# preethamam/AutomaticPanoramicImageStitching-AutoPanoStitch-MATLAB

Measured on AMD Instinct MI355X. Metric: MPix/s end-to-end stitch (SIFT->blend), 64x4K images, higher is better.
Workload: dtype f32; 1 GPU

## Files before the change

### automaticpanoramicimagestitching-autopanostitch-matlab_amd/csrc/sift.hip

```cpp
#include <algorithm>
#include <cmath>
#include <cstring>
#include <vector>

#include "aps_internal.h"
#include "select_dev.h"

namespace aps {

constexpr int kBorder = 5;
constexpr int kMaxInterp = 5;
constexpr int kOriBins = 36;
constexpr float kFix = 1048576.0f;

__device__ __forceinline__ long long to_fix(float v) { return (long long)(int)rintf(v * kFix); }
constexpr float kFltEps = 1.1920928955078125e-07f;

constexpr int kMaxViews = APS_SIFT_MAX_VIEWS;
constexpr int kViewShift = 44;
static_assert(kMaxViews <= 16, "the view takes 4 bits of the key");
struct ViewImgs {
    const uint8_t* p[kMaxViews];
};

// ... 195 lines not shown
        const int uc = live ? u : 0;
        const int seg = uc / (IH / 2), p = uc - seg * (IH / 2), xb = seg * 8;
        const f32x2* src = reinterpret_cast<const f32x2*>(&s_in[p * IP2 + 2 * (OFF + xb)]);
        f32x2 v[8 + 2 * R], acc[8];
#pragma unroll
        for (int j = 0; j < 8 + 2 * R; ++j) v[j] = src[j];
#pragma unroll
        for (int j = 0; j < 8; ++j) acc[j] = f32x2{0.f, 0.f};
        static_for<0, 2 * R + 1>([&](auto T) {
            constexpr int t = decltype(T)::value;
#pragma unroll
            for (int j = 0; j < 8; ++j) pk_tap<t>(acc[j], gk, v[j + t]);
        });
        if (one_buf) __syncthreads();
        float* d0 = &s_row[(2 * p) * RPITCH + xb];
        if (live) {
#pragma unroll
            for (int j = 0; j < 8; ++j) {
                d0[j] = acc[j].x;
                d0[RPITCH + j] = acc[j].y;
            }
        }
    }
    __syncthreads();
    for (int u = tid; u < (TW / 2) * (kTH / 4); u += NT) {
        const int lx = 2 * (u & (TW / 2 - 1)), yb = (u / (TW / 2)) * 4;
        f32x2 v[4 + 2 * R], acc[4];
#pragma unroll
        for (int j = 0; j < 4 + 2 * R; ++j) v[j] = *reinterpret_cast<const f32x2*>(&s_row[(yb + j) * RPITCH + lx]);
#pragma unroll
        for (int j = 0; j < 4; ++j) acc[j] = f32x2{0.f, 0.f};
        static_for<0, 2 * R + 1>([&](auto T) {
            constexpr int t = decltype(T)::value;
#pragma unroll
            for (int j = 0; j < 4; ++j) pk_tap<t>(acc[j], gk, v[j + t]);
        });
        const int gx = x0 + lx;
        if (gx + 1 < w && (w & 1) == 0) {
#pragma unroll
            for (int j = 0; j < 4; ++j) {
                const int gy = y0 + yb + j;
                if (gy < h) *reinterpret_cast<f32x2*>(&out[(size_t)gy * w + gx]) = acc[j];
            }
        } else if (gx < w) {
#pragma unroll
            for (int j = 0; j < 4; ++j) {
                const int gy = y0 + yb + j;
                if (gy < h) {
                    out[(size_t)gy * w + gx] = acc[j].x;
                    if (gx + 1 < w) out[(size_t)gy * w + gx + 1] = acc[j].y;
                }
            }
        }
        if (dec && (gx >> 1) < dw) {
#pragma unroll
            for (int j = 0; j < 4; j += 2) {
                const int dy = (y0 + yb + j) >> 1;
                if (dy < dh) dec[(size_t)dy * dw + (gx >> 1)] = acc[j].x;
            }
        }
    }
}

template <int R, int TW = kTW, int NT = 256>
__global__ __launch_bounds__(NT) void blur_kernel(const float* __restrict__ in_, int h, int w, GaussK gk,
                                                   float* __restrict__ out_, float* __restrict__ dec_, int dh, int dw,
                                                   size_t pitch, size_t dpitch) {
    const float* __restrict__ in = in_ + blockIdx.z * pitch;
    float* __restrict__ out = out_ + blockIdx.z * pitch;
    float* __restrict__ dec = dec_ ? dec_ + blockIdx.z * dpitch : nullptr;
    constexpr int RP = (R + 3) & ~3;
    constexpr int IW = TW + 2 * RP, IH = kTH + 2 * R, NV = IW / 4;
    static_assert(IH % 2 == 0 && kTH % 4 == 0, "row pairs");
    constexpr int IP2 = 2 * IW + 4;
    constexpr int RPITCH = TW + 2;
    static_assert((IP2 / 4) % 2 == 1, "pitch");
    static_assert(IH * RPITCH <= (IH / 2) * IP2, "the row-pass result fits the tile's buffer");
    __shared__ __attribute__((aligned(16))) float s_in[(IH / 2) * IP2];
    __shared__ __attribute__((aligned(16))) float s_row_own[kBlurOneBuffer<R> ? 1 : IH * RPITCH];
    float* const s_row = kBlurOneBuffer<R> ? s_in : s_row_own;
    const int x0 = blockIdx.x * TW, y0 = blockIdx.y * kTH;
    const int tid = threadIdx.x;
    const bool vec_ok = (w & 3) == 0 && (reinterpret_cast<uintptr_t>(in) & 15) == 0;
    constexpr int NPF = (IH * NV + NT - 1) / NT;
    float4 pf[NPF];
    const bool interior = vec_ok && x0 >= RP && x0 + TW + RP <= w && y0 >= R && y0 + kTH + R <= h;
    if (interior) {
        const float* base = in + ((size_t)(y0 - R) * w + (x0 - RP));
#pragma unroll
        for (int q = 0; q < NPF; ++q) {
            const int e = tid + NT * q;
            const int ec = e < IH * NV ? e : IH * NV - 1;
            const int ly = ec / NV, v = ec - ly * NV;
            pf[q] = *reinterpret_cast<const float4*>(base + (unsigned)(ly * w + 4 * v));
        }
    } else {
#pragma unroll
        for (int q = 0; q < NPF; ++q) {
            const int e = tid + NT * q;
            const int ec = e < IH * NV ? e : IH * NV - 1;
            const int ly = ec / NV, v = ec - ly * NV;
            const int gy = reflect101(y0 + ly - R, h), gx = x0 - RP + 4 * v;
            const float* row = in + (size_t)gy * w;
            if (vec_ok && gx >= 0 && gx + 3 < w) {
                pf[q] = *reinterpret_cast<const float4*>(row + gx);
            } else {
                pf[q].x = row[reflect101(gx, w)];
                pf[q].y = row[reflect101(gx + 1, w)];
                pf[q].z = row[reflect101(gx + 2, w)];
                pf[q].w = row[reflect101(gx + 3, w)];
            }
        }
    }
#pragma unroll
    for (int q = 0; q < NPF; ++q) {
        const int e = tid + NT * q;
        if (e < IH * NV) {
            const int ly = e / NV, v = e - ly * NV;
            float* dst = &s_in[(ly >> 1) * IP2 + 8 * v + (ly & 1)];
            dst[0] = pf[q].x;
            dst[2] = pf[q].y;
            dst[4] = pf[q].z;
            dst[6] = pf[q].w;
        }
    }
    blur_tile_passes<R, TW, NT>(s_in, s_row, gk, x0, y0, h, w, out, dec, dh, dw);
}

__global__ __launch_bounds__(256) void gray_u8_kernel(ViewImgs imgs, int h, int w, int c, int layout,
                                                      uint8_t* __restrict__ gray_, size_t gpitch) {
    const uint8_t* __restrict__ img = imgs.p[blockIdx.z];
    uint8_t* __restrict__ gray = gray_ + blockIdx.z * gpitch;
    const int x4 = (blockIdx.x * 256 + threadIdx.x) * 4, y = blockIdx.y;
    if (x4 >= w) return;
    uint8_t g[4];
    const bool fast = c == 3 && layout == APS_IMG_U8_HWC && (w & 3) == 0 && (reinterpret_cast<uintptr_t>(img) & 3) == 0;
    if (fast) {
        const uint32_t* p = reinterpret_cast<const uint32_t*>(img + ((size_t)y * w + x4) * 3);
        const uint32_t a = p[0], b = p[1], d_ = p[2];
        const uint8_t ch[12] = {(uint8_t)a, (uint8_t)(a >> 8), (uint8_t)(a >> 16), (uint8_t)(a >> 24), (uint8_t)b, (uint8_t)(b >> 8),
                                (uint8_t)(b >> 16), (uint8_t)(b >> 24), (uint8_t)d_, (uint8_t)(d_ >> 8), (uint8_t)(d_ >> 16), (uint8_t)(d_ >> 24)};
#pragma unroll
        for (int k = 0; k < 4; ++k) {
            const double d = 0.298936021293775 * ch[3 * k] + 0.587043074451121 * ch[3 * k + 1] + 0.114020904255103 * ch[3 * k + 2];
            g[k] = (uint8_t)(float)floor(d + 0.5);
        }
        *reinterpret_cast<uint32_t*>(gray + (size_t)y * w + x4) = g[0] | ((uint32_t)g[1] << 8) | ((uint32_t)g[2] << 16) | ((uint32_t)g[3] << 24);
        return;
    }
    for (int k = 0; k < 4 && x4 + k < w; ++k) {
        const int x = x4 + k;
        float v;
        if (c == 1) {
            v = (float)(layout == APS_IMG_U8_HWC ? img[(size_t)y * w + x] : img[(size_t)x * h + y]);
        } else {
            uint8_t ch[3];
#pragma unroll
            for (int q = 0; q < 3; ++q)
                ch[q] = layout == APS_IMG_U8_HWC ? img[((size_t)y * w + x) * 3 + q] : img[(size_t)q * h * w + (size_t)x * h + y];
            const double d = 0.298936021293775 * ch[0] + 0.587043074451121 * ch[1] + 0.114020904255103 * ch[2];
            v = (float)floor(d + 0.5);
        }
        gray[(size_t)y * w + x] = (uint8_t)v;
    }
}

template <int R>
__global__ __launch_bounds__(256) void blur_base_kernel(const uint8_t* __restrict__ gray_, size_t gpitch, int sh, int sw,
                                                        GaussK gk, float* __restrict__ out_, size_t pitch) {
    const uint8_t* __restrict__ gray = gray_ + blockIdx.z * gpitch;
    float* __restrict__ out = out_ + blockIdx.z * pitch;
    constexpr int RP = (R + 3) & ~3;
    constexpr int IW = kTW + 2 * RP, IH = kTH + 2 * R, NV = IW / 4;
    constexpr int IP2 = 2 * IW + 4;
    constexpr int RPITCH = kTW + 2;
    constexpr int GW = IW / 2 + 3, GH = IH / 2 + 3;
    __shared__ __attribute__((aligned(16))) float s_in[(IH / 2) * IP2];
    __shared__ __attribute__((aligned(16))) float s_row_own[kBlurOneBuffer<R> ? 1 : IH * RPITCH];
    float* const s_row = kBlurOneBuffer<R> ? s_in : s_row_own;
    __shared__ float s_g[GH][GW + 1];
    static_assert(GH * IW <= IH * RPITCH && IW % 4 == 0, "the horizontally interpolated gray rows fit the row-pass buffer");
    __shared__ __attribute__((aligned(16))) float s_h_own[kBlurOneBuffer<R> ? GH * IW : 4];
    const int h = 2 * sh, w = 2 * sw;
    const int x0 = blockIdx.x * kTW, y0 = blockIdx.y * kTH;
    const int tid = threadIdx.x;
    const int lo_x = max(x0 - RP, 0), lo_y = max(y0 - R, 0);
    const int cx0 = max((lo_x + 1) / 2 - 1, 0), cy0 = max((lo_y + 1) / 2 - 1, 0);
    for (int e = tid; e < GH * GW; e += 256) {
        const int ly = e / GW, lx = e - ly * GW;
        const int y = min(cy0 + ly, sh - 1), x = min(cx0 + lx, sw - 1);
        s_g[ly][lx] = (float)gray[(size_t)y * sw + x];
    }
    __shared__ int s_ci[IW + IH][2];
    __shared__ float s_cf[IW + IH];
    if (tid < IW + IH) {
        const bool col = tid < IW;
        const int n = col ? sw : sh, c0 = col ? cx0 : cy0, lim = col ? GW : GH;
        const int p = col ? reflect101(x0 - RP + tid, w) : reflect101(y0 + (tid - IW) - R, h);
        float f = ((float)p + 0.5f) * 0.5f - 0.5f;
        int s0 = (int)floorf(f);
        f -= (float)s0;
        if (s0 < 0) {
            s0 = 0;
            f = 0;
        }
        if (s0 >= n - 1) {
            s0 = n - 1;
            f = 0;
        }
        const int s1 = s0 + 1 < n ? s0 + 1 : n - 1;
        s_ci[tid][0] = min(max(s0 - c0, 0), lim - 1);
        s_ci[tid][1] = min(max(s1 - c0, 0), lim - 1);
        s_cf[tid] = f;
    }
    __syncthreads();
    float* const s_h = kBlurOneBuffer<R> ? s_h_own : s_row;
    for (int e = tid; e < GH * IW; e += 256) {
        const int gy = e / IW, cx = e - gy * IW;
        const float a1 = s_cf[cx], a0 = 1.0f - a1;
        const float* r = s_g[gy];
        s_h[gy * IW + cx] = r[s_ci[cx][0]] * a0 + r[s_ci[cx][1]] * a1;
    }
    __syncthreads();
    for (int e = tid; e < IH * NV; e += 256) {
        const int ly = e / NV, v = e - ly * NV;
        const float b1 = s_cf[IW + ly], b0 = 1.0f - b1;
        const float4 h0 = *reinterpret_cast<const float4*>(&s_h[s_ci[IW + ly][0] * IW + 4 * v]);
        const float4 h1 = *reinterpret_cast<const float4*>(&s_h[s_ci[IW + ly][1] * IW + 4 * v]);
        float* dst = &s_in[(ly >> 1) * IP2 + 8 * v + (ly & 1)];
        dst[0] = h0.x * b0 + h1.x * b1;
        dst[2] = h0.y * b0 + h1.y * b1;
        dst[4] = h0.z * b0 + h1.z * b1;
        dst[6] = h0.w * b0 + h1.w * b1;
    }
    blur_tile_passes<R>(s_in, s_row, gk, x0, y0, h, w, out, nullptr, 0, 0);
}

__global__ void blur_row_generic(const float* __restrict__ in_, int h, int w, GaussK gk, float* __restrict__ out_, size_t pitch) {
    const float* __restrict__ in = in_ + blockIdx.z * pitch;
    float* __restrict__ out = out_ + blockIdx.z * pitch;
    const int x = blockIdx.x * blockDim.x + threadIdx.x, y = blockIdx.y;
    if (x >= w) return;
    const int r = gk.n / 2;
    float acc = 0.f;
    for (int t = 0; t < gk.n; ++t) acc = fmaf(gk.k[t], in[(size_t)y * w + reflect101(x + t - r, w)], acc);
    out[(size_t)y * w + x] = acc;
}
__global__ void blur_col_generic(const float* __restrict__ tmp_, int h, int w, GaussK gk, float* __restrict__ out_, size_t pitch) {
    const float* __restrict__ tmp = tmp_ + blockIdx.z * pitch;
    float* __restrict__ out = out_ + blockIdx.z * pitch;
    const int x = blockIdx.x * blockDim.x + threadIdx.x, y = blockIdx.y;
    if (x >= w) return;
    const int r = gk.n / 2;
    float acc = 0.f;
    for (int t = 0; t < gk.n; ++t) acc = fmaf(gk.k[t], tmp[(size_t)reflect101(y + t - r, h) * w + x], acc);
    out[(size_t)y * w + x] = acc;
}

struct OctaveDesc {
    const float* G[8];
    int w, h;
};

struct KpRec {
    unsigned long long key;
    float xc, xr, xi, contr;
};

#define AT(L, rr, cc) (od.G[(L) + 1][(size_t)(rr) * w + (cc)] - od.G[(L)][(size_t)(rr) * w + (cc)])

__device__ bool adjust_extremum(const OctaveDesc& od, int nl, int o, int layer, int r, int c, float contr_thr,
                                float edge_thr, KpRec& kp) {
    const int w = od.w, h = od.h;
    const float img_scale = 1.0f / 255.0f, deriv_scale = img_scale * 0.5f, second_scale = img_scale,
                cross_scale = img_scale * 0.25f;
    float xi = 0, xr = 0, xc = 0;
    int i = 0;
    for (; i < kMaxInterp; ++i) {
        const int im = layer, pv = layer - 1, nx = layer + 1;
        const float dD0 = (AT(im, r, c + 1) - AT(im, r, c - 1)) * deriv_scale;
        const float dD1 = (AT(im, r + 1, c) - AT(im, r - 1, c)) * deriv_scale;
        const float dD2 = (AT(nx, r, c) - AT(pv, r, c)) * deriv_scale;
        const float v2 = AT(im, r, c) * 2.0f;
        const float dxx = (AT(im, r, c + 1) + AT(im, r, c - 1) - v2) * second_scale;
        const float dyy = (AT(im, r + 1, c) + AT(im, r - 1, c) - v2) * second_scale;
        const float dss = (AT(nx, r, c) + AT(pv, r, c) - v2) * second_scale;
        const float dxy = (AT(im, r + 1, c + 1) - AT(im, r + 1, c - 1) - AT(im, r - 1, c + 1) + AT(im, r - 1, c - 1)) * cross_scale;
        const float dxs = (AT(nx, r, c + 1) - AT(nx, r, c - 1) - AT(pv, r, c + 1) + AT(pv, r, c - 1)) * cross_scale;
        const float dys = (AT(nx, r + 1, c) - AT(nx, r - 1, c) - AT(pv, r + 1, c) + AT(pv, r - 1, c)) * cross_scale;
        float A[3][4] = {{dxx, dxy, dxs, dD0}, {dxy, dyy, dys, dD1}, {dxs, dys, dss, dD2}};
        bool singular = false;
#pragma unroll
        for (int col = 0; col < 3; ++col) {
            if (singular) break;
            int piv = col;
#pragma unroll
            for (int row = col + 1; row < 3; ++row)
                if (fabsf(A[row][col]) > fabsf(A[piv][col])) piv = row;
            if (fabsf(A[piv][col]) < kFltEps) {
                singular = true;
                break;
            }
            if (piv != col) {
#pragma unroll
                for (int e = 0; e < 4; ++e) {
                    const float t = A[piv][e];
                    A[piv][e] = A[col][e];
                    A[col][e] = t;
                }
            }
            const float d = -1.0f / A[col][col];
#pragma unroll
            for (int row = col + 1; row < 3; ++row) {
                const float alpha = A[row][col] * d;
#pragma unroll
                for (int e = col + 1; e < 4; ++e) A[row][e] = fmaf(alpha, A[col][e], A[row][e]);
            }
// ... 176 lines not shown
        for (int p = 0; p < ND; ++p) {
#pragma unroll
            for (int k = 0; k < 2; ++k) {
                wmax[p % 3][k] = fmaxf(fmaxf(hm[a][p][k], hm[b][p][k]), hm[c][p][k]);
                wmin[p % 3][k] = fminf(fminf(hn[a][p][k], hn[b][p][k]), hn[c][p][k]);
            }
            if (p < 2) continue;
            const int layer = p - 1;
#pragma unroll
            for (int k = 0; k < 2; ++k) {
                const float val = dc[b][layer - 1][k];
                const float mx = fmaxf(fmaxf(wmax[0][k], wmax[1][k]), wmax[2][k]);
                const float mn = fminf(fminf(wmin[0][k], wmin[1][k]), wmin[2][k]);
                const bool pass = (k ? ok1 : ok0) && fabsf(val) > thr && ((val > 0 && val >= mx) || (val < 0 && val <= mn));
                emit(pass, layer, r, c0 + k);
            }
        }
    };
    using I0 = std::integral_constant<int, 0>;
    using I1 = std::integral_constant<int, 1>;
    using I2 = std::integral_constant<int, 2>;
    fetch(I0{}, rc0 - 1);
    fetch(I1{}, rc0);
    fetch(I2{}, rc0 + 1);
    reduce_row(I0{});
    fetch(I0{}, rc0 + 2);
    reduce_row(I1{});
    fetch(I1{}, rc0 + 3);
    for (int r = rc0; r < rc1; r += 3) {
        reduce_row(I2{});
        fetch(I2{}, r + 4);
        test_row(I0{}, I1{}, I2{}, r);
        if (r + 1 >= rc1) break;
        reduce_row(I0{});
        fetch(I0{}, r + 5);
        test_row(I1{}, I2{}, I0{}, r + 1);
        if (r + 2 >= rc1) break;
        reduce_row(I1{});
        fetch(I1{}, r + 6);
        test_row(I2{}, I0{}, I1{}, r + 2);
    }
    if (qn == 0) return;
    const int n_loc = min(qn, kWCells);
    unsigned int base = 0;
    if (lane == 0) base = atomicAdd(count, (unsigned int)n_loc);
    base = __builtin_amdgcn_readfirstlane(base);
    __builtin_amdgcn_wave_barrier();
    for (int e = lane; e < n_loc; e += 64) {
        const unsigned int slot = base + e;
        if (slot < cap) cells[slot] = s_cells[wave][e];
    }
}

__global__ void refine_kernel(const PyrTable* __restrict__ pt, const unsigned long long* __restrict__ cells,
                              const unsigned int* __restrict__ n_cells, unsigned int cells_cap, float contr_thr,
                              float edge_thr, KpRec* __restrict__ recs, unsigned int* __restrict__ count,
                              unsigned int cap) {
    const unsigned int i = blockIdx.x * blockDim.x + threadIdx.x, view = blockIdx.y;
    const unsigned int n = min(n_cells[2 * view], cells_cap);
    if (i >= n) return;
    const unsigned long long key = cells[(size_t)view * cells_cap + i];
    const int o = key_octave(key), layer = (int)((key >> 32) & 0xff), r = (int)((key >> 16) & 0xffff),
              c = (int)(key & 0xffff);
    KpRec kp;
    if (!adjust_extremum(pt[view].oct[o], pt[view].nl, o, layer, r, c, contr_thr, edge_thr, kp)) return;
    kp.key |= (unsigned long long)view << kViewShift;
    const unsigned int slot = atomicAdd(count + 2 * view, 1u);
    if (slot < cap) recs[(size_t)view * cap + slot] = kp;
}

__device__ __forceinline__ float kp_scale(float sigma, int layer, float xi, int nl) {
    return sigma * my_exp2(((float)layer + xi) / (float)nl);
}

__global__ __launch_bounds__(256) void orient_kernel(const PyrTable* __restrict__ pt,
                                                     const KpRec* __restrict__ kps, unsigned int n,
                                                     unsigned int* __restrict__ ori_count,
                                                     float* __restrict__ ori_angle ,
                                                     unsigned char* __restrict__ ori_bin ) {
    __shared__ unsigned long long s_hist[4][kOriBins];
    __shared__ float s_h[4][kOriBins + 4];
    const int wv = threadIdx.x >> 6, lane = threadIdx.x & 63;
    const unsigned int ki = blockIdx.x * 4 + wv;
    const bool active = ki < n;
    if (lane < kOriBins) s_hist[wv][lane] = 0ull;
    __syncthreads();
    int o = 0, layer = 1, r0 = 0, c0 = 0, view = 0;
    float xi = 0;
    if (active) {
        const KpRec kp = kps[ki];
        view = key_view(kp.key);
        o = key_octave(kp.key);
        layer = (int)((kp.key >> 32) & 0xff);
        r0 = (int)((kp.key >> 16) & 0xffff);
        c0 = (int)(kp.key & 0xffff);
        xi = kp.xi;
    }
    pt += view;
    const OctaveDesc& od = pt->oct[o];
    const __attribute__((address_space(1))) float* g = (const __attribute__((address_space(1))) float*)od.G[layer];
    const int w = od.w, h = od.h;
    const float scl = kp_scale(pt->sigma, layer, xi, pt->nl);
    const int radius = (int)rintf(4.5f * scl);
    const float sig = 1.5f * scl;
    const float expf_scale = -1.0f / (2.0f * sig * sig);
    const int side = 2 * radius + 1;
    if (active) {
        for (int s = lane; s < side * side; s += 64) {
            const int i = s / side - radius, j = s % side - radius;
            const int y = r0 + i, x = c0 + j;
            if (y <= 0 || y >= h - 1 || x <= 0 || x >= w - 1) continue;
            const int ctr = y * w + x;
            const float dx = g[ctr + 1] - g[ctr - 1];
            const float dy = g[ctr - w] - g[ctr + w];
            const float wgt = my_exp((float)(i * i + j * j) * expf_scale);
            const float ori = fast_atan2_deg(dy, dx);
            const float mag = sqrtf(dx * dx + dy * dy);
            int bin = (int)rintf(((float)kOriBins / 360.0f) * ori);
            if (bin >= kOriBins) bin -= kOriBins;
            if (bin < 0) bin += kOriBins;
            const long long q = to_fix(wgt * mag);
            atomicAdd(&s_hist[wv][bin], (unsigned long long)q);
        }
    }
    __syncthreads();
    if (lane < kOriBins) s_h[wv][lane + 2] = (float)(long long)s_hist[wv][lane] * (1.0f / kFix);
    __syncthreads();
    if (lane < 2) {
        s_h[wv][lane] = s_h[wv][kOriBins + lane];
        s_h[wv][kOriBins + 2 + lane] = s_h[wv][2 + lane];
    }
    __syncthreads();
    float hv = 0.f;
    if (lane < kOriBins)
        hv = (s_h[wv][lane] + s_h[wv][lane + 4]) * (1.0f / 16.0f) + (s_h[wv][lane + 1] + s_h[wv][lane + 3]) * (4.0f / 16.0f) +
             s_h[wv][lane + 2] * (6.0f / 16.0f);
    __syncthreads();
    if (lane < kOriBins) s_h[wv][lane] = hv;
    __syncthreads();
    if (active) {
        float omax = lane < kOriBins ? s_h[wv][lane] : -INFINITY;
#pragma unroll
        for (int off = 32; off > 0; off >>= 1) omax = fmaxf(omax, __shfl_xor(omax, off));
        const float thr = omax * 0.8f;
        bool peak = false;
        float angle = 0.f;
        if (lane < kOriBins) {
            const int j = lane;
            const int l = j > 0 ? j - 1 : kOriBins - 1, r2 = j < kOriBins - 1 ? j + 1 : 0;
            const float hj = s_h[wv][j], hl = s_h[wv][l], hr = s_h[wv][r2];
            if (hj > hl && hj > hr && hj >= thr) {
                peak = true;
                float bin = (float)j + 0.5f * (hl - hr) / (hl - 2.0f * hj + hr);
                bin = bin < 0 ? (float)kOriBins + bin : (bin >= (float)kOriBins ? bin - (float)kOriBins : bin);
                angle = 360.0f - (360.0f / (float)kOriBins) * bin;
                if (fabsf(angle - 360.0f) < kFltEps) angle = 0.0f;
            }
        }
        const unsigned long long pm = __ballot(peak);
        if (peak) {
            const unsigned int cnt = (unsigned int)__popcll(pm & ((1ull << lane) - 1ull));
            ori_angle[(size_t)ki * kOriBins + cnt] = angle;
            ori_bin[(size_t)ki * kOriBins + cnt] = (unsigned char)lane;
        }
        if (lane == 0) ori_count[ki] = (unsigned int)__popcll(pm);
    }
}

struct OrientedKp {
    unsigned int kp;
    float angle;
};

__global__ void expand_oriented_kernel(const unsigned int* __restrict__ ori_count,
                                       const unsigned int* __restrict__ ori_pos,
                                       const float* __restrict__ ori_angle, unsigned int n,
                                       OrientedKp* __restrict__ out) {
    const unsigned int i = blockIdx.x * blockDim.x + threadIdx.x;
    if (i >= n) return;
    const unsigned int c = ori_count[i], p = ori_pos[i];
    for (unsigned int e = 0; e < c; ++e) {
        out[p + e].kp = i;
        out[p + e].angle = ori_angle[(size_t)i * kOriBins + e];
    }
}

__device__ __forceinline__ float octave_step(int o) { return ldexpf(1.0f, o) * 0.5f; }
__device__ __forceinline__ float sift_pt(int base, float offset) { return (float)base + offset; }
__device__ __forceinline__ double sift_loc(float pt, float step) { return (double)(pt * step) + 1.0; }

__global__ __launch_bounds__(256) void sift_contr_key_kernel(const KpRec* __restrict__ kps, const OrientedKp* __restrict__ oks,
                                                             unsigned int n, unsigned long long* __restrict__ keys,
                                                             unsigned int* __restrict__ vals) {
    const unsigned int i = blockIdx.x * 256 + threadIdx.x;
    if (i >= n) return;
    keys[i] = strength_key_f32(kps[oks[i].kp].contr);
    vals[i] = i;
}

__global__ __launch_bounds__(256) void sift_uniform_key_kernel(const KpRec* __restrict__ kps, const OrientedKp* __restrict__ oks,
                                                               unsigned int n, int H, int W, int rows, int cols,
                                                               unsigned long long* __restrict__ keys, unsigned int* __restrict__ vals) {
    const unsigned int i = blockIdx.x * 256 + threadIdx.x;
    if (i >= n) return;
    const KpRec kp = kps[oks[i].kp];
    const float step = octave_step(key_octave(kp.key));
    const double x = sift_loc(sift_pt((int)(kp.key & 0xffff), kp.xc), step), y = sift_loc(sift_pt((int)((kp.key >> 16) & 0xffff), kp.xr), step);
    const int px = min(max((int)floor(x) - 1, 0), W - 1), py = min(max((int)floor(y) - 1, 0), H - 1);
    keys[i] = (unsigned long long)uniform_cell(py, px, H, W, rows, cols) << kSegmentShift | strength_key_f32(kp.contr);
    vals[i] = i;
}

struct ViewDst {
    float* desc;
    double* loc;
    float* aux;
    unsigned int row0;
};
constexpr int kD = 4, kN = 8, kHistLen = (kD + 2) * (kD + 2) * (kN + 2);
constexpr int kDescQueue = 512;

__global__ __launch_bounds__(256) void descr_kernel(const PyrTable* __restrict__ pt,
                                                    const KpRec* __restrict__ kps,
                                                    const OrientedKp* __restrict__ oks, unsigned int n_out,
                                                    const ViewDst* __restrict__ dst, int desc_layout, int64_t ldd, int64_t ldl) {
    __shared__ unsigned long long s_hist[4][kHistLen];
    __shared__ __attribute__((aligned(16))) float s_raw[4][128];
    __shared__ int s_queue[4][kDescQueue];
    const int wv = threadIdx.x >> 6, lane = threadIdx.x & 63;
    const unsigned int oi = blockIdx.x * 4 + wv;
    const bool active = oi < n_out;
    for (int e = lane; e < kHistLen; e += 64) s_hist[wv][e] = 0ull;
    __syncthreads();
    int o = 0, layer = 1, r0 = 0, c0 = 0, view = 0;
    float xc = 0, xr = 0, xi = 0, contr = 0, kangle = 0;
    if (active) {
        const OrientedKp ok = oks[oi];
        const KpRec kp = kps[ok.kp];
        view = key_view(kp.key);
        o = key_octave(kp.key);
        layer = (int)((kp.key >> 32) & 0xff);
        r0 = (int)((kp.key >> 16) & 0xffff);
        c0 = (int)(kp.key & 0xffff);
        xc = kp.xc;
        xr = kp.xr;
        xi = kp.xi;
        contr = kp.contr;
        kangle = ok.angle;
    }
    pt += view;
    const OctaveDesc& od = pt->oct[o];
    const __attribute__((address_space(1))) float* g = (const __attribute__((address_space(1))) float*)od.G[layer];
    const int w = od.w, h = od.h;
    const float scl = kp_scale(pt->sigma, layer, xi, pt->nl);
    float ori = 360.0f - kangle;
    if (fabsf(ori - 360.0f) < kFltEps) ori = 0.0f;
    const float ptx = sift_pt(c0, xc), pty = sift_pt(r0, xr);
    const int px = (int)rintf(ptx), py = (int)rintf(pty);
    float sin_t, cos_t;
    sincos_deg(ori, sin_t, cos_t);
    const float bins_per_deg = (float)kN / 360.0f;
    const float exp_scale = -1.0f / ((float)(kD * kD) * 0.5f);
    const float hist_width = 3.0f * scl;
    int radius = (int)rintf(hist_width * 1.4142135623730951f * (float)(kD + 1) * 0.5f);
    const int diag = (int)sqrt((double)w * w + (double)h * h);
    if (radius > diag) radius = diag;
    cos_t = cos_t / hist_width;
    sin_t = sin_t / hist_width;
    const int side = 2 * radius + 1;
    (void)side;
    auto accumulate = [&](int i, int j) __attribute__((always_inline)) {
        const float c_rot = (float)j * cos_t - (float)i * sin_t;
        const float r_rot = (float)j * sin_t + (float)i * cos_t;
        float rbin = r_rot + (float)(kD / 2) - 0.5f;
        float cbin = c_rot + (float)(kD / 2) - 0.5f;
        const int r = py + i, c = px + j;
        const int ctr = r * w + c;
        const float dx = g[ctr + 1] - g[ctr - 1];
        const float dy = g[ctr - w] - g[ctr + w];
        const float wgt = my_exp((c_rot * c_rot + r_rot * r_rot) * exp_scale);
        const float o_deg = fast_atan2_deg(dy, dx);
        const float mag = sqrtf(dx * dx + dy * dy) * wgt;
        float obin = (o_deg - ori) * bins_per_deg;
        const int rr0 = (int)floorf(rbin), cc0 = (int)floorf(cbin);
        int o0 = (int)floorf(obin);
        rbin -= (float)rr0;
        cbin -= (float)cc0;
        obin -= (float)o0;
        if (o0 < 0) o0 += kN;
        if (o0 >= kN) o0 -= kN;
        const float v_r1 = mag * rbin, v_r0 = mag - v_r1;
        const float v_rc11 = v_r1 * cbin, v_rc10 = v_r1 - v_rc11;
        const float v_rc01 = v_r0 * cbin, v_rc00 = v_r0 - v_rc01;
        const float v111 = v_rc11 * obin, v110 = v_rc11 - v111;
        const float v101 = v_rc10 * obin, v100 = v_rc10 - v101;
        const float v011 = v_rc01 * obin, v010 = v_rc01 - v011;
        const float v001 = v_rc00 * obin, v000 = v_rc00 - v001;
        const int idx = ((rr0 + 1) * (kD + 2) + cc0 + 1) * (kN + 2) + o0;
        unsigned long long* hb = &s_hist[wv][idx];
#define ADDQ(off, v) atomicAdd(hb + (off), (unsigned long long)to_fix(v))
        ADDQ(0, v000);
        ADDQ(1, v001);
        ADDQ(kN + 2, v010);
        ADDQ(kN + 3, v011);
        ADDQ((kD + 2) * (kN + 2), v100);
        ADDQ((kD + 2) * (kN + 2) + 1, v101);
        ADDQ((kD + 3) * (kN + 2), v110);
        ADDQ((kD + 3) * (kN + 2) + 1, v111);
#undef ADDQ
    };
    if (active) {
        int* q = s_queue[wv];
        int qn = 0;
        auto flush = [&]() __attribute__((always_inline)) {
            const int rounds = (qn + 63) >> 6;
            __builtin_amdgcn_wave_barrier();
            const int e0 = lane * rounds;
            int pk = q[min(e0, kDescQueue - 1)];
            for (int r = 0; r < rounds; ++r) {
                const int e = e0 + r;
                const int pk_next = q[min(e + 1, kDescQueue - 1)];
                if (e < qn) accumulate(pk >> 16, (int)(short)(pk & 0xffff));
                pk = pk_next;
            }
            __builtin_amdgcn_wave_barrier();
            qn = 0;
        };
        auto passes = [&](int i, int j) __attribute__((always_inline)) {
            const float c_rot = (float)j * cos_t - (float)i * sin_t;
            const float r_rot = (float)j * sin_t + (float)i * cos_t;
            const float rbin = r_rot + (float)(kD / 2) - 0.5f;
            const float cbin = c_rot + (float)(kD / 2) - 0.5f;
            const int r = py + i, c = px + j;
            return j >= -radius && j <= radius && rbin > -1 && rbin < kD && cbin > -1 && cbin < kD && r > 0 && r < h - 1 && c > 0 && c < w - 1;
        };
        bool plain = radius > 63 || fabsf(sin_t) < 1e-4f || fabsf(cos_t) < 1e-4f;
        int jl_[2] = {0, 0}, len_[2] = {0, 0};
        if (!plain) {
            bool bad = false;
#pragma unroll
            for (int half = 0; half < 2; ++half) {
                const int i = -radius + lane + 64 * half;
                const bool row_ok = i <= radius && py + i > 0 && py + i < h - 1;
                const float fi = (float)i;
                float lo = fmaxf(-(float)radius, (float)(1 - px)), hi = fminf((float)radius, (float)(w - 2 - px));
                auto clip = [&](float a, float lo_v, float hi_v) __attribute__((always_inline)) {
                    const float p0 = lo_v / a, p1 = hi_v / a;
                    lo = fmaxf(lo, fminf(p0, p1));
                    hi = fminf(hi, fmaxf(p0, p1));
                };
                clip(sin_t, -2.5f - fi * cos_t, 2.5f - fi * cos_t);
                clip(cos_t, -2.5f + fi * sin_t, 2.5f + fi * sin_t);
                const int gl = (int)ceilf(lo), gh = (int)floorf(hi);
                int jl = 0x7fffffff, jh = -0x7fffffff;
#pragma unroll
                for (int dlt = 2; dlt >= -2; --dlt)
                    if (passes(i, gl + dlt)) jl = gl + dlt;
#pragma unroll
                for (int dlt = -2; dlt <= 2; ++dlt)
                    if (passes(i, gh + dlt)) jh = gh + dlt;
                const bool none = jl > jh;
                bool good;
                if (none)
                    good = gl > gh;
                else
                    good = !passes(i, jl - 1) && !passes(i, jh + 1) && passes(i, (jl + jh) / 2) && jl >= gl - 2 && jh <= gh + 2;
                bad = bad || (row_ok && !good);
                jl_[half] = jl;
                len_[half] = (row_ok && !none) ? jh - jl + 1 : 0;
            }
            plain = __any(bad) != 0;
        }
        if (!plain) {
#pragma unroll
            for (int half = 0; half < 2; ++half) {
                unsigned long long rows_m = __ballot(len_[half] > 0);
                while (rows_m) {
                    const int l = __ffsll((long long)rows_m) - 1;
                    rows_m &= rows_m - 1ull;
                    const int rj = __builtin_amdgcn_readlane(jl_[half], l), rn = __builtin_amdgcn_readlane(len_[half], l);
                    const int ri = -radius + l + 64 * half;
                    for (int t0 = 0; t0 < rn; t0 += 64) {
                        const int cnt = min(64, rn - t0);
                        if (lane < cnt) q[qn + lane] = (ri << 16) | ((rj + t0 + lane) & 0xffff);
                        qn += cnt;
                        if (qn > kDescQueue - 64) flush();
                    }
                }
            }
        } else {
            for (int i = -radius; i <= radius; ++i) {
                for (int j0 = -radius; j0 <= radius; j0 += 64) {
                    const int j = j0 + lane;
                    const bool pass = passes(i, j);
                    const unsigned long long m = __ballot(pass);
                    if (m == 0ull) continue;
                    if (pass) q[qn + __popcll(m & ((1ull << lane) - 1ull))] = (i << 16) | (j & 0xffff);
                    qn += __popcll(m);
                    if (qn > kDescQueue - 64) flush();
                }
            }
        }
        if (qn > 0) flush();
    }
    __syncthreads();
#pragma unroll
    for (int half = 0; half < 2; ++half) {
        const int e = lane + 64 * half;
        const int k = e & 7, ij = e >> 3, i = ij >> 2, j = ij & 3;
        const int idx = ((i + 1) * (kD + 2) + (j + 1)) * (kN + 2);
        long long v = (long long)s_hist[wv][idx + k];
        if (k < 2) v += (long long)s_hist[wv][idx + kN + k];
        s_raw[wv][e] = (float)v * (1.0f / kFix);
    }
    __syncthreads();
    if (!active) return;
    auto sumsq = [&]() __attribute__((always_inline)) {
        float a = 0;
#pragma unroll 4
        for (int k4 = 0; k4 < 32; ++k4) {
            const float4 v = *reinterpret_cast<const float4*>(&s_raw[wv][4 * k4]);
            a = fmaf(v.x, v.x, a);
            a = fmaf(v.y, v.y, a);
            a = fmaf(v.z, v.z, a);
            a = fmaf(v.w, v.w, a);
        }
        return a;
    };
    float nrm2 = sumsq();
    const float thr = sqrtf(nrm2) * 0.2f;
    float clip[2];
#pragma unroll
    for (int half = 0; half < 2; ++half) {
        const float v0 = s_raw[wv][lane + 64 * half];
        clip[half] = v0 < thr ? v0 : thr;
    }
    __builtin_amdgcn_wave_barrier();
    s_raw[wv][lane] = clip[0];
    s_raw[wv][lane + 64] = clip[1];
    __builtin_amdgcn_wave_barrier();
    nrm2 = sumsq();
    const float sn = sqrtf(nrm2);
    const float scale = 512.0f / (sn > kFltEps ? sn : kFltEps);
    float qv[2];
#pragma unroll
    for (int half = 0; half < 2; ++half) {
        float v = rintf(clip[half] * scale);
        qv[half] = v < 0 ? 0 : (v > 255 ? 255 : v);
    }
    __builtin_amdgcn_wave_barrier();
    s_raw[wv][lane] = qv[0];
    s_raw[wv][lane + 64] = qv[1];
    __builtin_amdgcn_wave_barrier();
    const float qq = sumsq();
    const float inv = sqrtf(qq);
    const ViewDst vd = dst[view];
    const size_t row = oi - vd.row0;
    __attribute__((address_space(1))) float* desc = (__attribute__((address_space(1))) float*)vd.desc;
#pragma unroll
    for (int half = 0; half < 2; ++half) {
        const int e = lane + 64 * half;
        const float outv = inv > 0 ? qv[half] / inv : 0.0f;
        if (desc_layout == APS_ROWMAJOR)
            desc[row * ldd + e] = outv;
        else
            desc[(size_t)e * ldd + row] = outv;
    }
    if (lane == 0) {
        const float s = octave_step(o);
        vd.loc[row] = sift_loc(ptx, s);
        vd.loc[ldl + row] = sift_loc(pty, s);
        if (vd.aux) {
            vd.aux[row * 4 + 0] = scl * s * 2.0f;
            vd.aux[row * 4 + 1] = kangle;
            vd.aux[row * 4 + 2] = contr;
            vd.aux[row * 4 + 3] = (float)(o + 256 * layer);
        }
    }
}

static GaussK make_gauss(double sigma) {
    GaussK g;
    int n = (int)std::lrint(sigma * 8.0 + 1.0) | 1;
    if (n > 63) n = 63;
    const double s2 = -0.5 / (sigma * sigma);
    double sum = 0;
    for (int i = 0; i < n; ++i) {
        const double x = i - (n - 1) * 0.5;
        g.k[i] = (float)std::exp(s2 * x * x);
        sum += g.k[i];
    }
    sum = 1.0 / sum;
    for (int i = 0; i < n; ++i) g.k[i] = (float)(g.k[i] * sum);
    g.n = n;
    return g;
}

static size_t view_pitch(int w, int h) { return ((size_t)w * h + 3) & ~(size_t)3; }

// ... 453 lines not shown
```

Baseline: 3291 MPix/s.

## Pair-row tile loads, fast interior upsample, wave-local barriers in SIFT kernels

```diff
diff --git a/automaticpanoramicimagestitching-autopanostitch-matlab_amd/csrc/sift.hip b/automaticpanoramicimagestitching-autopanostitch-matlab_amd/csrc/sift.hip
--- a/automaticpanoramicimagestitching-autopanostitch-matlab_amd/csrc/sift.hip
+++ b/automaticpanoramicimagestitching-autopanostitch-matlab_amd/csrc/sift.hip
@@ -301,46 +301,47 @@
     const int x0 = blockIdx.x * TW, y0 = blockIdx.y * kTH;
     const int tid = threadIdx.x;
     const bool vec_ok = (w & 3) == 0 && (reinterpret_cast<uintptr_t>(in) & 15) == 0;
-    constexpr int NPF = (IH * NV + NT - 1) / NT;
-    float4 pf[NPF];
+    constexpr int NIT = (IH / 2) * NV, NPF = (NIT + NT - 1) / NT;
+    float4 pa[NPF], pb[NPF];
     const bool interior = vec_ok && x0 >= RP && x0 + TW + RP <= w && y0 >= R && y0 + kTH + R <= h;
     if (interior) {
         const float* base = in + ((size_t)(y0 - R) * w + (x0 - RP));
 #pragma unroll
         for (int q = 0; q < NPF; ++q) {
             const int e = tid + NT * q;
-            const int ec = e < IH * NV ? e : IH * NV - 1;
-            const int ly = ec / NV, v = ec - ly * NV;
-            pf[q] = *reinterpret_cast<const float4*>(base + (unsigned)(ly * w + 4 * v));
+            const int ec = e < NIT ? e : NIT - 1;
+            const int p = ec / NV, v = ec - p * NV;
+            const unsigned off = (unsigned)(2 * p * w + 4 * v);
+            pa[q] = *reinterpret_cast<const float4*>(base + off);
+            pb[q] = *reinterpret_cast<const float4*>(base + (off + (unsigned)w));
         }
     } else {
 #pragma unroll
         for (int q = 0; q < NPF; ++q) {
             const int e = tid + NT * q;
-            const int ec = e < IH * NV ? e : IH * NV - 1;
-            const int ly = ec / NV, v = ec - ly * NV;
-            const int gy = reflect101(y0 + ly - R, h), gx = x0 - RP + 4 * v;
-            const float* row = in + (size_t)gy * w;
+            const int ec = e < NIT ? e : NIT - 1;
+            const int p = ec / NV, v = ec - p * NV;
+            const int gx = x0 - RP + 4 * v;
+            const float* row_a = in + (size_t)reflect101(y0 + 2 * p - R, h) * w;
+            const float* row_b = in + (size_t)reflect101(y0 + 2 * p + 1 - R, h) * w;
             if (vec_ok && gx >= 0 && gx + 3 < w) {
-                pf[q] = *reinterpret_cast<const float4*>(row + gx);
+                pa[q] = *reinterpret_cast<const float4*>(row_a + gx);
+                pb[q] = *reinterpret_cast<const float4*>(row_b + gx);
             } else {
-                pf[q].x = row[reflect101(gx, w)];
-                pf[q].y = row[reflect101(gx + 1, w)];
-                pf[q].z = row[reflect101(gx + 2, w)];
-                pf[q].w = row[reflect101(gx + 3, w)];
+                const int g0 = reflect101(gx, w), g1 = reflect101(gx + 1, w), g2 = reflect101(gx + 2, w), g3 = reflect101(gx + 3, w);
+                pa[q] = make_float4(row_a[g0], row_a[g1], row_a[g2], row_a[g3]);
+                pb[q] = make_float4(row_b[g0], row_b[g1], row_b[g2], row_b[g3]);
             }
         }
     }
 #pragma unroll
     for (int q = 0; q < NPF; ++q) {
         const int e = tid + NT * q;
-        if (e < IH * NV) {
-            const int ly = e / NV, v = e - ly * NV;
-            float* dst = &s_in[(ly >> 1) * IP2 + 8 * v + (ly & 1)];
-            dst[0] = pf[q].x;
-            dst[2] = pf[q].y;
-            dst[4] = pf[q].z;
-            dst[6] = pf[q].w;
+        if (e < NIT) {
+            const int p = e / NV, v = e - p * NV;
+            float4* dst = reinterpret_cast<float4*>(&s_in[p * IP2 + 8 * v]);
+            dst[0] = make_float4(pa[q].x, pb[q].x, pa[q].y, pb[q].y);
+            dst[1] = make_float4(pa[q].z, pb[q].z, pa[q].w, pb[q].w);
         }
     }
     blur_tile_passes<R, TW, NT>(s_in, s_row, gk, x0, y0, h, w, out, dec, dh, dw);
@@ -412,7 +413,8 @@
     }
     __shared__ int s_ci[IW + IH][2];
     __shared__ float s_cf[IW + IH];
-    if (tid < IW + IH) {
+    const bool interior = x0 >= RP && x0 + kTW + RP < w && y0 >= R && y0 + kTH + R < h;
+    if (!interior && tid < IW + IH) {
         const bool col = tid < IW;
         const int n = col ? sw : sh, c0 = col ? cx0 : cy0, lim = col ? GW : GH;
         const int p = col ? reflect101(x0 - RP + tid, w) : reflect101(y0 + (tid - IW) - R, h);
@@ -434,24 +436,52 @@
     }
     __syncthreads();
     float* const s_h = kBlurOneBuffer<R> ? s_h_own : s_row;
-    for (int e = tid; e < GH * IW; e += 256) {
-        const int gy = e / IW, cx = e - gy * IW;
-        const float a1 = s_cf[cx], a0 = 1.0f - a1;
-        const float* r = s_g[gy];
-        s_h[gy * IW + cx] = r[s_ci[cx][0]] * a0 + r[s_ci[cx][1]] * a1;
-    }
-    __syncthreads();
-    for (int e = tid; e < IH * NV; e += 256) {
-        const int ly = e / NV, v = e - ly * NV;
-        const float b1 = s_cf[IW + ly], b0 = 1.0f - b1;
-        const float4 h0 = *reinterpret_cast<const float4*>(&s_h[s_ci[IW + ly][0] * IW + 4 * v]);
-        const float4 h1 = *reinterpret_cast<const float4*>(&s_h[s_ci[IW + ly][1] * IW + 4 * v]);
-        float* dst = &s_in[(ly >> 1) * IP2 + 8 * v + (ly & 1)];
-        dst[0] = h0.x * b0 + h1.x * b1;
-        dst[2] = h0.y * b0 + h1.y * b1;
-        dst[4] = h0.z * b0 + h1.z * b1;
-        dst[6] = h0.w * b0 + h1.w * b1;
-    }
+    const int ry = y0 - R - 1 - 2 * cy0;
+    auto interpolate = [&](auto INTERIOR) __attribute__((always_inline)) {
+        auto terms = [&](int k, int u, int& i0, int& i1, float& f1) __attribute__((always_inline)) {
+            if constexpr (decltype(INTERIOR)::value) {
+                i0 = u >> 1;
+                i1 = i0 + 1;
+                f1 = (u & 1) ? 0.75f : 0.25f;
+            } else {
+                i0 = s_ci[k][0];
+                i1 = s_ci[k][1];
+                f1 = s_cf[k];
+            }
+        };
+        for (int e = tid; e < GH * IW; e += 256) {
+            const int gy = e / IW, cx = e - gy * IW;
+            int i0, i1;
+            float a1;
+            terms(cx, cx + 1, i0, i1, a1);
+            const float a0 = 1.0f - a1;
+            const float* r = s_g[gy];
+            s_h[gy * IW + cx] = r[i0] * a0 + r[i1] * a1;
+        }
+        __syncthreads();
+        for (int e = tid; e < (IH / 2) * NV; e += 256) {
+            const int p = e / NV, v = e - p * NV;
+            float4 res[2];
+#pragma unroll
+            for (int half = 0; half < 2; ++half) {
+                const int ly = 2 * p + half;
+                int j0, j1;
+                float b1;
+                terms(IW + ly, ly + ry, j0, j1, b1);
+                const float b0 = 1.0f - b1;
+                const float4 h0 = *reinterpret_cast<const float4*>(&s_h[j0 * IW + 4 * v]);
+                const float4 h1 = *reinterpret_cast<const float4*>(&s_h[j1 * IW + 4 * v]);
+                res[half] = make_float4(h0.x * b0 + h1.x * b1, h0.y * b0 + h1.y * b1, h0.z * b0 + h1.z * b1, h0.w * b0 + h1.w * b1);
+            }
+            float4* dst = reinterpret_cast<float4*>(&s_in[p * IP2 + 8 * v]);
+            dst[0] = make_float4(res[0].x, res[1].x, res[0].y, res[1].y);
+            dst[1] = make_float4(res[0].z, res[1].z, res[0].w, res[1].w);
+        }
+    };
+    if (interior)
+        interpolate(std::true_type{});
+    else
+        interpolate(std::false_type{});
     blur_tile_passes<R>(s_in, s_row, gk, x0, y0, h, w, out, nullptr, 0, 0);
 }
 
@@ -794,20 +824,13 @@
     __shared__ float s_h[4][kOriBins + 4];
     const int wv = threadIdx.x >> 6, lane = threadIdx.x & 63;
     const unsigned int ki = blockIdx.x * 4 + wv;
-    const bool active = ki < n;
+    if (ki >= n) return;
     if (lane < kOriBins) s_hist[wv][lane] = 0ull;
-    __syncthreads();
-    int o = 0, layer = 1, r0 = 0, c0 = 0, view = 0;
-    float xi = 0;
-    if (active) {
-        const KpRec kp = kps[ki];
-        view = key_view(kp.key);
-        o = key_octave(kp.key);
-        layer = (int)((kp.key >> 32) & 0xff);
-        r0 = (int)((kp.key >> 16) & 0xffff);
-        c0 = (int)(kp.key & 0xffff);
-        xi = kp.xi;
-    }
+    __builtin_amdgcn_wave_barrier();
+    const KpRec kp = kps[ki];
+    const int view = key_view(kp.key), o = key_octave(kp.key), layer = (int)((kp.key >> 32) & 0xff);
+    const int r0 = (int)((kp.key >> 16) & 0xffff), c0 = (int)(kp.key & 0xffff);
+    const float xi = kp.xi;
     pt += view;
     const OctaveDesc& od = pt->oct[o];
     const __attribute__((address_space(1))) float* g = (const __attribute__((address_space(1))) float*)od.G[layer];
@@ -817,66 +840,62 @@
     const float sig = 1.5f * scl;
     const float expf_scale = -1.0f / (2.0f * sig * sig);
     const int side = 2 * radius + 1;
-    if (active) {
-        for (int s = lane; s < side * side; s += 64) {
-            const int i = s / side - radius, j = s % side - radius;
-            const int y = r0 + i, x = c0 + j;
-            if (y <= 0 || y >= h - 1 || x <= 0 || x >= w - 1) continue;
-            const int ctr = y * w + x;
-            const float dx = g[ctr + 1] - g[ctr - 1];
-            const float dy = g[ctr - w] - g[ctr + w];
-            const float wgt = my_exp((float)(i * i + j * j) * expf_scale);
-            const float ori = fast_atan2_deg(dy, dx);
-            const float mag = sqrtf(dx * dx + dy * dy);
-            int bin = (int)rintf(((float)kOriBins / 360.0f) * ori);
-            if (bin >= kOriBins) bin -= kOriBins;
-            if (bin < 0) bin += kOriBins;
-            const long long q = to_fix(wgt * mag);
-            atomicAdd(&s_hist[wv][bin], (unsigned long long)q);
-        }
-    }
-    __syncthreads();
+    for (int s = lane; s < side * side; s += 64) {
+        const int i = s / side - radius, j = s % side - radius;
+        const int y = r0 + i, x = c0 + j;
+        if (y <= 0 || y >= h - 1 || x <= 0 || x >= w - 1) continue;
+        const int ctr = y * w + x;
+        const float dx = g[ctr + 1] - g[ctr - 1];
+        const float dy = g[ctr - w] - g[ctr + w];
+        const float wgt = my_exp((float)(i * i + j * j) * expf_scale);
+        const float ori = fast_atan2_deg(dy, dx);
+        const float mag = sqrtf(dx * dx + dy * dy);
+        int bin = (int)rintf(((float)kOriBins / 360.0f) * ori);
+        if (bin >= kOriBins) bin -= kOriBins;
+        if (bin < 0) bin += kOriBins;
+        const long long q = to_fix(wgt * mag);
+        atomicAdd(&s_hist[wv][bin], (unsigned long long)q);
+    }
+    __builtin_amdgcn_wave_barrier();
     if (lane < kOriBins) s_h[wv][lane + 2] = (float)(long long)s_hist[wv][lane] * (1.0f / kFix);
-    __syncthreads();
+    __builtin_amdgcn_wave_barrier();
     if (lane < 2) {
         s_h[wv][lane] = s_h[wv][kOriBins + lane];
         s_h[wv][kOriBins + 2 + lane] = s_h[wv][2 + lane];
     }
-    __syncthreads();
+    __builtin_amdgcn_wave_barrier();
     float hv = 0.f;
     if (lane < kOriBins)
         hv = (s_h[wv][lane] + s_h[wv][lane + 4]) * (1.0f / 16.0f) + (s_h[wv][lane + 1] + s_h[wv][lane + 3]) * (4.0f / 16.0f) +
              s_h[wv][lane + 2] * (6.0f / 16.0f);
-    __syncthreads();
+    __builtin_amdgcn_wave_barrier();
     if (lane < kOriBins) s_h[wv][lane] = hv;
-    __syncthreads();
-    if (active) {
-        float omax = lane < kOriBins ? s_h[wv][lane] : -INFINITY;
-#pragma unroll
-        for (int off = 32; off > 0; off >>= 1) omax = fmaxf(omax, __shfl_xor(omax, off));
-        const float thr = omax * 0.8f;
-        bool peak = false;
-        float angle = 0.f;
-        if (lane < kOriBins) {
-            const int j = lane;
-            const int l = j > 0 ? j - 1 : kOriBins - 1, r2 = j < kOriBins - 1 ? j + 1 : 0;
-            const float hj = s_h[wv][j], hl = s_h[wv][l], hr = s_h[wv][r2];
-            if (hj > hl && hj > hr && hj >= thr) {
-                peak = true;
-                float bin = (float)j + 0.5f * (hl - hr) / (hl - 2.0f * hj + hr);
-                bin = bin < 0 ? (float)kOriBins + bin : (bin >= (float)kOriBins ? bin - (float)kOriBins : bin);
-                angle = 360.0f - (360.0f / (float)kOriBins) * bin;
-                if (fabsf(angle - 360.0f) < kFltEps) angle = 0.0f;
-            }
-        }
-        const unsigned long long pm = __ballot(peak);
-        if (peak) {
-            const unsigned int cnt = (unsigned int)__popcll(pm & ((1ull << lane) - 1ull));
-            ori_angle[(size_t)ki * kOriBins + cnt] = angle;
-            ori_bin[(size_t)ki * kOriBins + cnt] = (unsigned char)lane;
-        }
-        if (lane == 0) ori_count[ki] = (unsigned int)__popcll(pm);
-    }
+    __builtin_amdgcn_wave_barrier();
+    float omax = lane < kOriBins ? s_h[wv][lane] : -INFINITY;
+#pragma unroll
+    for (int off = 32; off > 0; off >>= 1) omax = fmaxf(omax, __shfl_xor(omax, off));
+    const float thr = omax * 0.8f;
+    bool peak = false;
+    float angle = 0.f;
+    if (lane < kOriBins) {
+        const int j = lane;
+        const int l = j > 0 ? j - 1 : kOriBins - 1, r2 = j < kOriBins - 1 ? j + 1 : 0;
+        const float hj = s_h[wv][j], hl = s_h[wv][l], hr = s_h[wv][r2];
+        if (hj > hl && hj > hr && hj >= thr) {
+            peak = true;
+            float bin = (float)j + 0.5f * (hl - hr) / (hl - 2.0f * hj + hr);
+            bin = bin < 0 ? (float)kOriBins + bin : (bin >= (float)kOriBins ? bin - (float)kOriBins : bin);
+            angle = 360.0f - (360.0f / (float)kOriBins) * bin;
+            if (fabsf(angle - 360.0f) < kFltEps) angle = 0.0f;
+        }
+    }
+    const unsigned long long pm = __ballot(peak);
+    if (peak) {
+        const unsigned int cnt = (unsigned int)__popcll(pm & ((1ull << lane) - 1ull));
+        ori_angle[(size_t)ki * kOriBins + cnt] = angle;
+        ori_bin[(size_t)ki * kOriBins + cnt] = (unsigned char)lane;
+    }
+    if (lane == 0) ori_count[ki] = (unsigned int)__popcll(pm);
 }
 
 struct OrientedKp {
@@ -941,25 +960,14 @@
     __shared__ int s_queue[4][kDescQueue];
     const int wv = threadIdx.x >> 6, lane = threadIdx.x & 63;
     const unsigned int oi = blockIdx.x * 4 + wv;
-    const bool active = oi < n_out;
+    if (oi >= n_out) return;
     for (int e = lane; e < kHistLen; e += 64) s_hist[wv][e] = 0ull;
-    __syncthreads();
-    int o = 0, layer = 1, r0 = 0, c0 = 0, view = 0;
-    float xc = 0, xr = 0, xi = 0, contr = 0, kangle = 0;
-    if (active) {
-        const OrientedKp ok = oks[oi];
-        const KpRec kp = kps[ok.kp];
-        view = key_view(kp.key);
-        o = key_octave(kp.key);
-        layer = (int)((kp.key >> 32) & 0xff);
-        r0 = (int)((kp.key >> 16) & 0xffff);
-        c0 = (int)(kp.key & 0xffff);
-        xc = kp.xc;
-        xr = kp.xr;
-        xi = kp.xi;
-        contr = kp.contr;
-        kangle = ok.angle;
-    }
+    __builtin_amdgcn_wave_barrier();
+    const OrientedKp ok = oks[oi];
+    const KpRec kp = kps[ok.kp];
+    const int view = key_view(kp.key), o = key_octave(kp.key), layer = (int)((kp.key >> 32) & 0xff);
+    const int r0 = (int)((kp.key >> 16) & 0xffff), c0 = (int)(kp.key & 0xffff);
+    const float xc = kp.xc, xr = kp.xr, xi = kp.xi, contr = kp.contr, kangle = ok.angle;
     pt += view;
     const OctaveDesc& od = pt->oct[o];
     const __attribute__((address_space(1))) float* g = (const __attribute__((address_space(1))) float*)od.G[layer];
@@ -992,7 +1000,7 @@
         const float dy = g[ctr - w] - g[ctr + w];
         const float wgt = my_exp((c_rot * c_rot + r_rot * r_rot) * exp_scale);
         const float o_deg = fast_atan2_deg(dy, dx);
-        const float mag = sqrtf(dx * dx + dy * dy) * wgt;
+        const float mag = (sqrtf(dx * dx + dy * dy) * wgt) * kFix;
         float obin = (o_deg - ori) * bins_per_deg;
         const int rr0 = (int)floorf(rbin), cc0 = (int)floorf(cbin);
         int o0 = (int)floorf(obin);
@@ -1010,7 +1018,7 @@
         const float v001 = v_rc00 * obin, v000 = v_rc00 - v001;
         const int idx = ((rr0 + 1) * (kD + 2) + cc0 + 1) * (kN + 2) + o0;
         unsigned long long* hb = &s_hist[wv][idx];
-#define ADDQ(off, v) atomicAdd(hb + (off), (unsigned long long)to_fix(v))
+#define ADDQ(off, v) atomicAdd(hb + (off), (unsigned long long)(unsigned int)rintf(v))
         ADDQ(0, v000);
         ADDQ(1, v001);
         ADDQ(kN + 2, v010);
@@ -1021,7 +1029,7 @@
         ADDQ((kD + 3) * (kN + 2) + 1, v111);
 #undef ADDQ
     };
-    if (active) {
+    {
         int* q = s_queue[wv];
         int qn = 0;
         auto flush = [&]() __attribute__((always_inline)) {
@@ -1115,7 +1123,7 @@
         }
         if (qn > 0) flush();
     }
-    __syncthreads();
+    __builtin_amdgcn_wave_barrier();
 #pragma unroll
     for (int half = 0; half < 2; ++half) {
         const int e = lane + 64 * half;
@@ -1125,8 +1133,7 @@
         if (k < 2) v += (long long)s_hist[wv][idx + kN + k];
         s_raw[wv][e] = (float)v * (1.0f / kFix);
     }
-    __syncthreads();
-    if (!active) return;
+    __builtin_amdgcn_wave_barrier();
     auto sumsq = [&]() __attribute__((always_inline)) {
         float a = 0;
 #pragma unroll 4
```

Measured after the change: 3270 MPix/s. About the same (-0.6%).
